# danielwillemsen/alphazero-openspiel

Measured on NVIDIA B200. Metric: mcts_simulations_per_sec, higher is better.
Workload: dtype f64

## Files before the change

alphazero_openspiel_b200/csrc/az_engine.cu:

```cuda

#include <cuda_runtime.h>
#include <cuda_bf16.h>
#include <stdint.h>
#include <stdio.h>
#include <stdarg.h>
#include <string.h>
#include <math.h>
#include <new>
#include <vector>

#include "../../include/az_b200.h"
#include "az_games.cuh"

namespace az {

constexpr int PH_BEGIN = 6;
constexpr int PH_COMPACT = 7;
constexpr int BLOCK = 128;
#ifndef K_STEP_MIN_BLOCKS
#define K_STEP_MIN_BLOCKS 7
#endif

struct __align__(16) TreeHdr {
  uint64_t root_b0, root_b1;
  uint64_t pend_b0, pend_b1;
  int32_t root_node;
  int32_t alloc;
  int32_t sims_done;
  int32_t pend_node;
  int32_t pend_depth;
  int32_t pend_ply;
  int32_t root_ply;
  int32_t game_seq;
  uint8_t phase, half, err, uct;
  int32_t fast_sims;
  int32_t pad2[2];
};
static_assert(sizeof(TreeHdr) == 80, "TreeHdr size");

__device__ __forceinline__ St root_state(const TreeHdr& h) {
  St s;
  s.b0 = h.root_b0;
  s.b1 = h.root_b1;
  s.ply = h.root_ply;
  return s;
}
__device__ __forceinline__ St pend_state(const TreeHdr& h) {
  St s;
  s.b0 = h.pend_b0;
  s.b1 = h.pend_b1;
  s.ply = h.pend_ply;
  return s;
}
__device__ __forceinline__ void set_root(TreeHdr& h, const St& s) {
  h.root_b0 = s.b0;
  h.root_b1 = s.b1;
  h.root_ply = s.ply;
}
__device__ __forceinline__ void set_pend(TreeHdr& h, const St& s, int node, int depth) {
  h.pend_b0 = s.b0;
  h.pend_b1 = s.b1;
  h.pend_ply = s.ply;
  h.pend_node = node;
  h.pend_depth = depth;
}

struct __align__(16) VlPend {
  uint64_t b0, b1;
  int32_t node, depth, ply, valid;
};

struct ResignCfg {
  double threshold;
  int32_t permille;
  int32_t pad;
};
struct ResignTree {
  double rmin[2];
  int32_t game_seq;
  int32_t calib;
};

struct PlayoutCapCfg {
  int32_t fast_playouts;
  int32_t full_permille;
};

struct Node;
struct Params {
  TreeHdr* hdr;
  Node* nodes;
  int32_t* path;
  uint8_t* rec;
  unsigned long long* rec_count;
  unsigned long long* ctr;
  int* games_started;
  int* compact_list;
  int* compact_count;
  long long* dbg;
  VlPend* vl_pend;
  int vl_k;
  uint8_t* cache;
  unsigned long long cache_mask;
  uint32_t* cache_epoch;
  ResignCfg* resign_cfg;
  ResignTree* resign_tree;
  PlayoutCapCfg* pcap_cfg;
  const double* logtab;
  long long rec_cap;
  int max_games;
  int rec_stride;
  int n_trees, cap;
  int n_playouts, num_prob, noise_mode, eval_mode, eval_shift, max_sims, start_mod;
  int cycle_budget;
  uint32_t flags;
  uint64_t seed;
  double c_puct, keep, noise_w, alpha, temperature;
  Geo geo;
};

__device__ __forceinline__ int search_target(const Params& p, const TreeHdr& h) {
  return h.fast_sims ? h.fast_sims : p.n_playouts;
}

struct StepIO {
  const void* priors;
  const void* values;
  const double* noise;
  void* obs;
  int obs_format;
};

template <int G>
__device__ __forceinline__ unsigned group_mask() {
  if constexpr (G >= 32) {
    return 0xffffffffu;
  } else {
    const unsigned lane = threadIdx.x & 31u;
    return ((1u << G) - 1u) << (lane & ~(unsigned)(G - 1));
  }
}
template <int G, class T>
__device__ __forceinline__ T gshfl(unsigned m, T v, int src) { return __shfl_sync(m, v, src, G); }
template <int G, class T>
__device__ __forceinline__ T gshfl_xor(unsigned m, T v, int off) { return __shfl_xor_sync(m, v, off, G); }
template <int G>
__device__ __forceinline__ int gsum(unsigned m, int v) {
#pragma unroll
  for (int o = G / 2; o > 0; o >>= 1) v += __shfl_xor_sync(m, v, o, G);
  return v;
}
template <int G>
__device__ __forceinline__ double gsumd(unsigned m, double v) {
#pragma unroll
  for (int o = G / 2; o > 0; o >>= 1) v += __shfl_xor_sync(m, v, o, G);
  return v;
}
template <int G>
__device__ __forceinline__ int gscan_incl(unsigned m, int v, int lane) {
#pragma unroll
  for (int o = 1; o < G; o <<= 1) {
    const int t = __shfl_up_sync(m, v, o, G);
    if (lane >= o) v += t;
  }
  return v;
}
template <int G>
__device__ __forceinline__ void gargmax(unsigned m, double& v, int& i) {
#pragma unroll
  for (int o = G / 2; o > 0; o >>= 1) {
    const double ov = __shfl_xor_sync(m, v, o, G);
    const int oi = __shfl_xor_sync(m, i, o, G);
    if (oi != 0x7fffffff && (i == 0x7fffffff || ov > v || (ov == v && oi < i))) { v = ov; i = oi; }
  }
}

__device__ __forceinline__ void ctr_add(unsigned long long* s_ctr, int which, unsigned long long v) {
  if (v) atomicAdd(&s_ctr[which], v);
}

struct StepCtr {
  unsigned long long sims = 0, depth = 0, children = 0, exp = 0, legal = 0, term = 0;
  __device__ __forceinline__ void flush(unsigned long long* s_ctr, int alloc) const {
    atomicMax(&s_ctr[AZ_CTR_PEAK_NODES], (unsigned long long)alloc);
    ctr_add(s_ctr, AZ_CTR_SIMS, sims);
    ctr_add(s_ctr, AZ_CTR_DEPTH, depth);
    ctr_add(s_ctr, AZ_CTR_CHILDREN, children);
    ctr_add(s_ctr, AZ_CTR_EXPANSIONS, exp);
    ctr_add(s_ctr, AZ_CTR_LEGAL, legal);
    ctr_add(s_ctr, AZ_CTR_TERMINAL, term);
  }
};

__device__ __forceinline__ void flush_block_counters(const Params& p, const unsigned long long* s_ctr) {
  __syncthreads();
  if (threadIdx.x < AZ_CTR_COUNT && s_ctr[threadIdx.x]) {
    if (threadIdx.x == AZ_CTR_PEAK_NODES) atomicMax(&p.ctr[threadIdx.x], s_ctr[threadIdx.x]);
    else atomicAdd(&p.ctr[threadIdx.x], s_ctr[threadIdx.x]);
  }
}

__device__ __forceinline__ void arena_overflow(TreeHdr& h, int lane, unsigned long long* s_ctr) {
  h.err = 1;
  if (lane == 0) ctr_add(s_ctr, AZ_CTR_OVERFLOW, 1);
}

struct EvalKey {
  uint64_t k;
};
__device__ __forceinline__ EvalKey eval_key(const Params& p, const St& s) {
  EvalKey e;
  e.k = mix64(s.b0 ^ mix64(s.b1 ^ mix64(p.seed + (uint64_t)(s.ply & 1))));
  return e;
}
__device__ __forceinline__ double eval_prior(const Params& p, const StepIO& io, int tree, const EvalKey& ek, int a) {
  if (p.eval_mode == AZ_EVAL_EXTERNAL) {
    const size_t idx = (size_t)tree * p.geo.n_actions + a;
    return (p.flags & AZ_F_PRIORS_F64) ? ((const double*)io.priors)[idx] : (double)((const float*)io.priors)[idx];
  }
  if (p.eval_mode == AZ_EVAL_UNIFORM) return 1.0 / (double)p.geo.n_actions;
  if (p.eval_mode == AZ_EVAL_ROLLOUT) return 1.0;
  const uint64_t ha = mix64(ek.k + (uint64_t)(a + 1) * 0xD1B54A32D192ED03ULL);
  return (double)(1 + (int)((ha >> 40) & 0x3FF)) * exp2((double)-(10 + p.eval_shift));
}
template <class GM>
__device__ double rollout_value(const Params& p, St s, const EvalKey& ek) {
  const int mover = s.ply & 1;
  for (uint64_t j = 0;; ++j) {
    const int out = GM::outcome(s, p.geo);
    if (out >= 0) return out == 2 ? 0.0 : (out == mover ? 1.0 : -1.0);
    const typename GM::Legal lg = GM::legal(s, p.geo);
    const int n = GM::count(lg);
    const uint64_t r = mix64(ek.k + (j + 1) * 0x9E3779B97F4A7C15ULL);
    s = GM::apply(s, p.geo, GM::action_of(lg, s, p.geo, (int)(r % (uint64_t)n)));
  }
}
template <class GM>
__device__ __forceinline__ double eval_value(const Params& p, const StepIO& io, int tree, const EvalKey& ek, const St& s) {
  if (p.eval_mode == AZ_EVAL_EXTERNAL)
    return (p.flags & AZ_F_PRIORS_F64) ? ((const double*)io.values)[tree] : (double)((const float*)io.values)[tree];
  if (p.eval_mode == AZ_EVAL_UNIFORM) return 0.0;
  if (p.eval_mode == AZ_EVAL_ROLLOUT) return rollout_value<GM>(p, s, ek);
  return (double)((int)((ek.k >> 20) & 31) - 16) / 16.0;
}

struct CacheHead {
  uint64_t b0, b1;
  uint32_t tag;
  float value;
};
static_assert(sizeof(CacheHead) == 24, "CacheHead size");
template <class GM>
__host__ __device__ constexpr int cache_stride() {
  int s = 1;
  while (s < (int)sizeof(CacheHead) + 4 * GM::MAXC + 4) s *= 2;
  return s;
}
template <class GM>
__device__ __forceinline__ uint8_t* cache_slot(const Params& p, const St& s) {
  return p.cache + (size_t)(eval_key(p, s).k & p.cache_mask) * cache_stride<GM>();
}
template <class GM>
__device__ __forceinline__ const CacheHead* cache_find(const Params& p, const St& s) {
  const CacheHead* e = reinterpret_cast<const CacheHead*>(cache_slot<GM>(p, s));
  const uint32_t tag = (p.cache_epoch[0] << 1) | (uint32_t)(s.ply & 1);
  return (e->b0 == s.b0 && e->b1 == s.b1 && e->tag == tag) ? e : nullptr;
}
__device__ __forceinline__ const float* cache_priors(const CacheHead* e) { return reinterpret_cast<const float*>(e + 1); }

__device__ double gamma_draw(double alpha, uint64_t seed, uint64_t tree, uint64_t gseq, uint64_t ply, int child) {
  const double d = alpha + 1.0 - 1.0 / 3.0, c = 1.0 / sqrt(9.0 * d);
  for (int att = 0; att < 64; ++att) {
    const uint64_t base = (uint64_t)child * 256 + (uint64_t)att * 4;
    const uint64_t r0 = counter(seed, tree, gseq, ply, base + 0, 5);
    const uint64_t r1 = counter(seed, tree, gseq, ply, base + 1, 5);
    const uint64_t r2 = counter(seed, tree, gseq, ply, base + 2, 5);
    const double u0 = ((double)(r0 >> 11) + 1.0) * (1.0 / 9007199254740992.0);
    const double u1 = ((double)(r1 >> 11) + 0.5) * (1.0 / 9007199254740992.0);
    const double u2 = ((double)(r2 >> 11) + 1.0) * (1.0 / 9007199254740992.0);
    const double x = sqrt(-2.0 * log(u0)) * cospi(2.0 * u1);
    double v = 1.0 + c * x;
    if (v <= 0.0) continue;
    v = v * v * v;
    const uint64_t r3 = counter(seed, tree, gseq, ply, base + 3, 5);
    const double u3 = ((double)(r3 >> 11) + 1.0) * (1.0 / 9007199254740992.0);
    if (log(u3) < 0.5 * x * x + d - d * v + d * log(v)) return d * v * pow(u2, 1.0 / alpha);
  }
  return alpha;
}

template <class GM, int G>
__device__ __forceinline__ void write_obs(const Params& p, const StepIO& io, int tree, int lane, const St& s) {
  if (io.obs_format == AZ_OBS_NONE || io.obs == nullptr) return;
  const int n = p.geo.cells;
  const uint64_t pl0 = GM::plane(s, p.geo, 0), pl1 = GM::plane(s, p.geo, 1), pl2 = GM::plane(s, p.geo, 2);
  const int cur = s.ply & 1;
  if (io.obs_format == AZ_OBS_BF16_NHWC) {
    uint2* out = reinterpret_cast<uint2*>(io.obs) + (size_t)tree * n;
    const uint32_t one = 0x3F80u;
    for (int c = lane; c < n; c += G) {
      uint2 v;
      v.x = (((pl0 >> c) & 1ULL) ? one : 0u) | ((((pl1 >> c) & 1ULL) ? one : 0u) << 16);
      v.y = (((pl2 >> c) & 1ULL) ? one : 0u) | ((cur ? one : 0u) << 16);
      out[c] = v;
    }
  } else {
    float* out = reinterpret_cast<float*>(io.obs) + (size_t)tree * 4 * n;
    for (int i = lane; i < 4 * n; i += G) {
      const int ch = i / n, c = i - ch * n;
      const uint64_t pm = ch == 0 ? pl0 : (ch == 1 ? pl1 : pl2);
      out[i] = ch == 3 ? (float)cur : (float)((pm >> c) & 1ULL);
    }
  }
}

struct __align__(8) Node {
  uint2 nl;
  double q;
  double p;
};
static_assert(sizeof(Node) == 24, "Node size");
struct Arena {
  Node* nd;
  __device__ __forceinline__ uint2& nl(int i) const { return nd[i].nl; }
  __device__ __forceinline__ double& q(int i) const { return nd[i].q; }
  __device__ __forceinline__ double& p(int i) const { return nd[i].p; }
};
__device__ __forceinline__ Arena arena_of(const Params& p, int tree, int half) {
  Arena a;
  a.nd = p.nodes + ((size_t)tree * 2 + half) * (size_t)p.cap;
  return a;
}

template <int G>
__device__ __forceinline__ void backup_path(const Arena& a, const int32_t* path, int depth, double v_leaf, int lane) {
  for (int j = lane; j <= depth; j += G) {
    const int node = path[j];
    const double v = ((depth - j) & 1) ? -v_leaf : v_leaf;
    const uint2 nl = a.nl(node);
    const double q = a.q(node);
    a.q(node) = __ddiv_rn(__dadd_rn(__dmul_rn((double)nl.x, q), v), (double)(nl.x + 1u));
    a.nl(node).x = nl.x + 1u;
  }
}

template <class GM, int G>
__device__ __forceinline__ bool expand_node(const Params& p, const StepIO& io, const Arena& a, TreeHdr& h, int tree,
                                            int node, const St& s, int lane, unsigned gm, bool root_mix,
                                            const double* eta_lane , int* L_out,
// ... 373 lines not shown
      const double ret0 = out == 2 ? 0.0 : (out == 0 ? 1.0 : -1.0);
      emit_record<GM, G>(p, tree, h, s2, 1, -1, 0, 0, ret0, rmin0, rmin1, end, nullptr, nullptr, lane, gm, s_ctr);
    }
    end_game<GM, G>(p, h, tree, lane, gm, s_ctr, s2);
    return;
  }
  set_root(h, s2);
  if ((p.flags & AZ_F_KEEP_TREE) && nc > 0) {
    if (!(p.flags & AZ_F_EAGER_COMPACT) && (long long)h.alloc + (long long)(p.n_playouts + 1) * GM::MAXC <= (long long)p.cap) {
      h.root_node = fc + k;
      h.phase = PH_BEGIN;
      return;
    }
    h.pend_node = fc + k;
    h.phase = PH_COMPACT;
    if (lane == 0) p.compact_list[atomicAdd(p.compact_count, 1)] = tree;
    return;
  }
  fresh_tree<G>(p, h, tree, lane, gm);
  h.phase = PH_BEGIN;
}

template <class GM, int G>
__device__ __forceinline__ void expand_root(const Params& p, const StepIO& io, TreeHdr& h, int tree, int row, int lane,
                                            unsigned gm, unsigned long long* s_ctr, const float* cached) {
  const Arena a = arena_of(p, tree, h.half);
  const St s = root_state(h);
  const typename GM::Legal lg = GM::legal(s, p.geo);
  const int L = GM::count(lg);
  double eta[GM::SLOTS];
#pragma unroll
  for (int sl = 0; sl < GM::SLOTS; ++sl) eta[sl] = 0.0;
  if (p.noise_mode == AZ_NOISE_HOST) {
#pragma unroll
    for (int sl = 0; sl < GM::SLOTS; ++sl) {
      const int i = lane + sl * G;
      if (i < L) eta[sl] = io.noise[(size_t)tree * GM::MAXC + i];
    }
  } else if (p.noise_mode == AZ_NOISE_COUNTER) {
    double sum = 0.0;
    for (int i = 0; i < L; ++i) {
      const double u = (double)((counter(p.seed, tree, h.game_seq, s.ply, i, 1) >> 11) + 1ULL) *
                       (1.0 / 9007199254740992.0);
      sum = __dadd_rn(sum, u);
#pragma unroll
      for (int sl = 0; sl < GM::SLOTS; ++sl)
        if (i == lane + sl * G) eta[sl] = u;
    }
#pragma unroll
    for (int sl = 0; sl < GM::SLOTS; ++sl) eta[sl] = __ddiv_rn(eta[sl], sum);
  } else if (p.noise_mode == AZ_NOISE_DIRICHLET) {
    double sum = 0.0;
#pragma unroll
    for (int sl = 0; sl < GM::SLOTS; ++sl) {
      const int i = lane + sl * G;
      if (i < L) eta[sl] = gamma_draw(p.alpha, p.seed, tree, h.game_seq, s.ply, i);
      sum += eta[sl];
    }
    sum = gsumd<G>(gm, sum);
#pragma unroll
    for (int sl = 0; sl < GM::SLOTS; ++sl) eta[sl] = sum > 0.0 ? eta[sl] / sum : 1.0 / (double)L;
  }
  int L2 = 0;
  if (!expand_node<GM, G>(p, io, a, h, row, h.root_node, s, lane, gm, true, eta, &L2, cached)) arena_overflow(h, lane, s_ctr);
  h.phase = AZ_PH_RUN;
  if (lane == 0) ctr_add(s_ctr, AZ_CTR_ROOT_EVALS, 1);
}

template <class GM, int G, bool CACHE>
__device__ __forceinline__ bool begin_search(const Params& p, const StepIO& io, TreeHdr& h, int tree, int row, int lane,
                                             unsigned gm, unsigned long long* s_ctr) {
  h.sims_done = 0;
  h.phase = AZ_PH_RUN;
  h.fast_sims = 0;
  if (p.flags & AZ_F_PLAYOUT_CAP) {
    const PlayoutCapCfg c = *p.pcap_cfg;
    if ((int)(counter(p.seed, tree, h.game_seq, h.root_ply, 0, 7) % 1000ULL) >= c.full_permille) {
      h.fast_sims = c.fast_playouts;
      return false;
    }
  }
  if (p.noise_mode == AZ_NOISE_NONE) return false;
  const St s = root_state(h);
  const CacheHead* hit = CACHE && p.cache ? cache_find<GM>(p, s) : nullptr;
  if (hit) {
    expand_root<GM, G>(p, io, h, tree, row, lane, gm, s_ctr, cache_priors(hit));
    return false;
  }
  h.phase = AZ_PH_ROOT_EVAL;
  set_pend(h, s, h.root_node, 0);
  write_obs<GM, G>(p, io, row, lane, s);
  return true;
}

template <class GM, int G, void (*BACKUP)(const Arena&, const int32_t*, int, double, int)>
__device__ __forceinline__ void apply_leaf(const Params& p, const StepIO& io, const Arena& a, TreeHdr& h, int row, int node,
                                           const St& s, const int32_t* path, int depth, const CacheHead* cached, int lane,
                                           unsigned gm, unsigned long long* s_ctr, StepCtr& c) {
  int L = 0;
  if (!expand_node<GM, G>(p, io, a, h, row, node, s, lane, gm, false, nullptr, &L, cached ? cache_priors(cached) : nullptr))
    arena_overflow(h, lane, s_ctr);
  const double v = cached ? (double)cached->value : eval_value<GM>(p, io, row, eval_key(p, s), s);
  BACKUP(a, path, depth, -v, lane);
  __syncwarp(gm);
  h.sims_done += 1;
  c.sims += 1;
  c.depth += depth;
  c.exp += 1;
  c.legal += L;
  if (cached && lane == 0) ctr_add(s_ctr, AZ_CTR_CACHE_HITS, 1);
}

template <int G>
__device__ __forceinline__ void terminal_leaf(const Arena& a, TreeHdr& h, const int32_t* path, int depth, int out, int ply,
                                              int lane, unsigned gm, StepCtr& c) {
  backup_path<G>(a, path, depth, mover_return(out, ply), lane);
  __syncwarp(gm);
  h.sims_done += 1;
  c.sims += 1;
  c.depth += depth;
  c.term += 1;
}

template <class GM, bool UCT>
__global__ void __launch_bounds__(BLOCK, K_STEP_MIN_BLOCKS) k_step(const Params p, const StepIO io) {
  constexpr int G = GM::G;
  __shared__ int32_t s_path[BLOCK / G][GM::MAXD];
  __shared__ unsigned long long s_ctr[AZ_CTR_COUNT];
  if (threadIdx.x < AZ_CTR_COUNT) s_ctr[threadIdx.x] = 0ULL;
  __syncthreads();
  const int tree = (int)((blockIdx.x * (unsigned)BLOCK + threadIdx.x) / G);
  const int lane = threadIdx.x % G;
  if (p.cache && blockIdx.x == 0 && threadIdx.x == 0) p.cache_epoch[1] = p.cache_epoch[0];
  if (tree < p.n_trees) {
    const unsigned gm = group_mask<G>();
    int32_t* spath = s_path[threadIdx.x / G];
    int32_t* gpath = p.path + (size_t)tree * GM::MAXD;
    const long long t_start = p.dbg ? clock64() : 0;
    const long long t_begin = p.cycle_budget > 0 ? clock64() : 0;
    TreeHdr h = p.hdr[tree];
    const int phase_in = h.phase;
    long long t_consume = 0;
    StepCtr c;

    if (h.phase == AZ_PH_LEAF_EVAL) {
      apply_leaf<GM, G, backup_path<G>>(p, io, arena_of(p, tree, h.half), h, tree, h.pend_node, pend_state(h), gpath,
                                        h.pend_depth, nullptr, lane, gm, s_ctr, c);
      h.phase = AZ_PH_RUN;
    } else if (h.phase == AZ_PH_ROOT_EVAL) {
      expand_root<GM, G>(p, io, h, tree, tree, lane, gm, s_ctr, nullptr);
    }

    if (p.dbg) t_consume = clock64() - t_start;
    int sims_this_step = 0;
    bool advanced = false;
    for (;;) {
      if (h.phase == PH_BEGIN && begin_search<GM, G, true>(p, io, h, tree, tree, lane, gm, s_ctr)) break;
      if (h.phase != AZ_PH_RUN) {
        if (lane == 0) ctr_add(s_ctr, AZ_CTR_IDLE_SLOTS, 1);
        break;
      }
      if (h.sims_done >= search_target(p, h)) {
        if (advanced) {
          if (lane == 0) ctr_add(s_ctr, AZ_CTR_IDLE_SLOTS, 1);
          break;
        }
        finish_move<GM, G>(p, h, tree, lane, gm, s_ctr);
        advanced = true;
        continue;
      }
      if (p.max_sims > 0 && sims_this_step >= p.max_sims) {
        if (lane == 0) ctr_add(s_ctr, AZ_CTR_IDLE_SLOTS, 1);
        break;
      }
      if (p.cycle_budget > 0 && sims_this_step > 0) {
        const int over = gshfl<G>(gm, (int)(clock64() - t_begin > (long long)p.cycle_budget), 0);
        if (over) {
          if (lane == 0) ctr_add(s_ctr, AZ_CTR_IDLE_SLOTS, 1);
          break;
        }
      }
      const Arena a = arena_of(p, tree, h.half);
      St s = root_state(h);
      int node, depth;
      bool dovf = false;
      sim_select<GM, G, UCT>(p, a, h.root_node, s, node, depth, spath, lane, gm, c.children, dovf, h.uct != 0);
      if (dovf) {
        h.err = 1;
        h.phase = AZ_PH_ERROR;
        if (lane == 0) ctr_add(s_ctr, AZ_CTR_OVERFLOW, 1);
        break;
      }
      const int out = depth > 0 ? GM::outcome(s, p.geo) : -1;
      ++sims_this_step;
      if (out >= 0) {
        terminal_leaf<G>(a, h, spath, depth, out, s.ply, lane, gm, c);
        if (p.flags & AZ_F_MANUAL) {
          for (int j = lane; j <= depth; j += G) gpath[j] = spath[j];
          h.pend_depth = depth;
        }
        continue;
      }
      const CacheHead* hit = p.cache ? cache_find<GM>(p, s) : nullptr;
      if (hit) {
        apply_leaf<GM, G, backup_path<G>>(p, io, a, h, tree, node, s, spath, depth, hit, lane, gm, s_ctr, c);
        continue;
      }
      set_pend(h, s, node, depth);
      h.phase = AZ_PH_LEAF_EVAL;
      for (int j = lane; j <= depth; j += G) gpath[j] = spath[j];
      write_obs<GM, G>(p, io, tree, lane, s);
      break;
    }

    if (lane == 0) {
      p.hdr[tree] = h;
      if (p.dbg) {
        p.dbg[4 * tree + 0] = clock64() - t_start;
        p.dbg[4 * tree + 1] = phase_in;
        p.dbg[4 * tree + 2] = sims_this_step;
        p.dbg[4 * tree + 3] = t_consume * 2 + (advanced ? 1 : 0);
      }
      c.flush(s_ctr, h.alloc);
    }
  }
  flush_block_counters(p, s_ctr);
}

template <class GM>
__global__ void __launch_bounds__(BLOCK) k_cache_insert(const Params p, const StepIO io) {
  constexpr int G = GM::G;
  const int tree = (int)((blockIdx.x * (unsigned)BLOCK + threadIdx.x) / G);
  const int lane = threadIdx.x % G;
  if (tree >= p.n_trees) return;
  const TreeHdr& h = p.hdr[tree];
  if (h.phase != AZ_PH_LEAF_EVAL && h.phase != AZ_PH_ROOT_EVAL) return;
  const unsigned gm = group_mask<G>();
  const St s = pend_state(h);
  uint8_t* slot = cache_slot<GM>(p, s);
  unsigned* lock = reinterpret_cast<unsigned*>(slot + cache_stride<GM>() - 4);
  int got = 0;
  if (lane == 0) got = atomicCAS(lock, 0u, 1u) == 0u;
  if (!gshfl<G>(gm, got, 0)) return;
  const typename GM::Legal lg = GM::legal(s, p.geo);
  const int L = GM::count(lg);
  float* pri = reinterpret_cast<float*>(slot + sizeof(CacheHead));
  const float* row = (const float*)io.priors + (size_t)tree * p.geo.n_actions;
#pragma unroll
  for (int sl = 0; sl < GM::SLOTS; ++sl) {
    const int i = lane + sl * G;
    if (i < L) pri[i] = row[GM::action_of(lg, s, p.geo, i)];
  }
  if (lane == 0) {
    CacheHead e;
    e.b0 = s.b0;
    e.b1 = s.b1;
    e.tag = (p.cache_epoch[1] << 1) | (uint32_t)(s.ply & 1);
    e.value = ((const float*)io.values)[tree];
    *reinterpret_cast<CacheHead*>(slot) = e;
  }
  __threadfence();
  __syncwarp(gm);
  if (lane == 0) atomicExch(lock, 0u);
}

__global__ void k_cache_new_epoch(uint32_t* epoch) { epoch[0] += 1u; }

constexpr unsigned VL_MARK = 0xFFFFFF00u;

template <int G>
__device__ __forceinline__ void vl_apply(const Arena& a, const int32_t* path, int depth, int lane) {
  for (int j = lane; j <= depth; j += G) {
    const int node = path[j];
    const uint2 nl = a.nl(node);
    a.q(node) = ((double)nl.x * a.q(node) - 1.0) / (double)(nl.x + 1u);
    a.nl(node).x = nl.x + 1u;
  }
}
template <int G>
__device__ __forceinline__ void vl_backup(const Arena& a, const int32_t* path, int depth, double v_leaf, int lane) {
  for (int j = lane; j <= depth; j += G) {
    const int node = path[j];
    const double v = ((depth - j) & 1) ? -v_leaf : v_leaf;
    const uint2 nl = a.nl(node);
    a.q(node) = ((double)nl.x * a.q(node) + 1.0 + v) / (double)nl.x;
  }
}

template <class GM>
__global__ void __launch_bounds__(BLOCK, 4) k_step_vl(const Params p, const StepIO io) {
  constexpr int G = GM::G;
  __shared__ int32_t s_path[BLOCK / G][GM::MAXD];
  __shared__ unsigned long long s_ctr[AZ_CTR_COUNT];
  if (threadIdx.x < AZ_CTR_COUNT) s_ctr[threadIdx.x] = 0ULL;
  __syncthreads();
  const int tree = (int)((blockIdx.x * (unsigned)BLOCK + threadIdx.x) / G);
  const int lane = threadIdx.x % G;
  if (tree < p.n_trees) {
    const unsigned gm = group_mask<G>();
    const int K = p.vl_k;
    int32_t* spath = s_path[threadIdx.x / G];
    int32_t* gpaths = p.path + (size_t)tree * K * GM::MAXD;
    VlPend* pend = p.vl_pend + (size_t)tree * K;
    const int row0 = tree * K;
    TreeHdr h = p.hdr[tree];
    StepCtr c;

    if (h.phase == AZ_PH_LEAF_EVAL) {
      const Arena a = arena_of(p, tree, h.half);
      for (int slot = 0; slot < K; ++slot) {
        const VlPend pe = pend[slot];
        if (!pe.valid) continue;
        St s;
        s.b0 = pe.b0;
        s.b1 = pe.b1;
        s.ply = pe.ply;
        if (lane == 0) a.nl(pe.node).y = 0u;
        __syncwarp(gm);
        apply_leaf<GM, G, vl_backup<G>>(p, io, a, h, row0 + slot, pe.node, s, gpaths + (size_t)slot * GM::MAXD, pe.depth,
                                        nullptr, lane, gm, s_ctr, c);
        if (lane == 0) pend[slot].valid = 0;
      }
      h.phase = AZ_PH_RUN;
    } else if (h.phase == AZ_PH_ROOT_EVAL) {
      expand_root<GM, G>(p, io, h, tree, row0, lane, gm, s_ctr, nullptr);
    }

    int n_pending = 0, sims_this_step = 0;
    bool advanced = false;
    for (;;) {
      if (h.phase == PH_BEGIN && begin_search<GM, G, false>(p, io, h, tree, row0, lane, gm, s_ctr)) {
        n_pending = 1;
        break;
      }
      if (h.phase != AZ_PH_RUN) break;
      if (h.sims_done + n_pending >= search_target(p, h)) {
        if (n_pending > 0 || advanced) break;
        finish_move<GM, G>(p, h, tree, lane, gm, s_ctr);
        advanced = true;
        continue;
      }
      if (n_pending >= K) break;
      if (p.max_sims > 0 && sims_this_step >= p.max_sims + K) break;
      const Arena a = arena_of(p, tree, h.half);
      St s = root_state(h);
      int node, depth;
      bool dovf = false;
      sim_select<GM, G, false>(p, a, h.root_node, s, node, depth, spath, lane, gm, c.children, dovf, false);
      if (dovf) {
// ... 426 lines not shown
  for (int r = 0; r < rows; ++r) {
    c0 |= 1ULL << (r * cols);
    cl |= 1ULL << (r * cols + cols - 1);
  }
  g.notcol0 = g.all & ~c0;
  g.notcolL = g.all & ~cl;
  g.row0 = cols >= 64 ? ~0ULL : ((1ULL << cols) - 1ULL);
  g.rowL = g.row0 << ((rows - 1) * cols);
  return g;
}

static int check_game(int game_id, int rows, int cols) {
  if (game_id == AZ_GAME_CONNECT_FOUR) return 0;
  if (game_id != AZ_GAME_BREAKTHROUGH) return fail(-1, "unknown game_id %d", game_id);
  if (rows < 4 || cols < 2 || rows * cols > 64 || cols > 16)
    return fail(-1, "breakthrough %dx%d unsupported (need rows>=4, cols>=2, rows*cols<=64)", rows, cols);
  return 0;
}

template <class F>
static int dispatch_game(int game_id, F&& f) {
  if (game_id == AZ_GAME_CONNECT_FOUR) return f(C4());
  return f(BT());
}

static inline int compact_grid(int n_trees) {
  int grid = n_trees / 128 + 4;
  return grid > 296 ? 296 : grid;
}
static inline int groups_grid(int n_trees, int G, int block) { return (int)(((long long)n_trees * G + block - 1) / block); }

extern "C" {

const char* az_last_error(void) { return g_err; }
int az_version(void) { return 1; }

int az_create(const az_config* cfg_in, az_engine** out) {
  if (!cfg_in || !out) return fail(-1, "null argument");
  az_config cfg = *cfg_in;
  if (check_game(cfg.game_id, cfg.rows, cfg.cols)) return -1;
  if (cfg.game_id == AZ_GAME_CONNECT_FOUR) {
    cfg.rows = 6;
    cfg.cols = 7;
  }
  if (cfg.n_trees <= 0) return fail(-1, "n_trees must be positive");
  if (cfg.n_playouts <= 0) return fail(-1, "n_playouts must be positive");
  if (cfg.temperature <= 0.0) cfg.temperature = 1.0;
  if (cfg.dirichlet_alpha <= 0.0) cfg.dirichlet_alpha = 0.3;
  if (cfg.noise_weight == 0.0) cfg.noise_weight = 0.25;
  if (cfg.num_probabilistic_actions <= 0) cfg.num_probabilistic_actions = 1000;
  if (cfg.noise_mode < 0 || cfg.noise_mode > 3) return fail(-1, "bad noise_mode");
  if (cfg.eval_mode < 0 || cfg.eval_mode > 3) return fail(-1, "bad eval_mode");
  const int maxc = cfg.game_id == AZ_GAME_CONNECT_FOUR ? C4::MAXC : BT::MAXC;
  const int maxd = cfg.game_id == AZ_GAME_CONNECT_FOUR ? C4::MAXD : BT::MAXD;
  const int group = cfg.game_id == AZ_GAME_CONNECT_FOUR ? C4::G : BT::G;
  if (cfg.node_capacity <= 0) {
    const int branch = cfg.game_id == AZ_GAME_CONNECT_FOUR ? 7 : 3 * cfg.cols + 8;
    long long c = (long long)(cfg.n_playouts + 2) * branch * 8 + 64;
    if (c > (1 << 24) - 1) c = (1 << 24) - 1;
    cfg.node_capacity = (int)c;
  }
  if (cfg.node_capacity >= (1 << 24)) return fail(-1, "node_capacity must be < 2^24");
  if (cfg.leaves_per_tree <= 0 || !(cfg.flags & AZ_F_VIRTUAL_LOSS)) cfg.leaves_per_tree = 1;
  if (cfg.leaves_per_tree > 64) return fail(-1, "leaves_per_tree must be <= 64");
  if ((cfg.flags & AZ_F_VIRTUAL_LOSS) && (cfg.flags & (AZ_F_MANUAL | AZ_F_UCT)))
    return fail(-1, "AZ_F_VIRTUAL_LOSS is a batched self-play mode (no AZ_F_MANUAL / AZ_F_UCT)");
  if ((cfg.flags & AZ_F_RESIGN) && (cfg.flags & AZ_F_MANUAL))
    return fail(-1, "AZ_F_RESIGN is a batched self-play mode: with AZ_F_MANUAL the host decides the moves");
  if ((cfg.flags & AZ_F_PLAYOUT_CAP) && (cfg.flags & AZ_F_MANUAL))
    return fail(-1, "AZ_F_PLAYOUT_CAP is a batched self-play mode: with AZ_F_MANUAL the host starts the searches");
  if (cfg.record_capacity <= 0) cfg.record_capacity = cfg.n_trees * 64 < (1 << 20) ? (1 << 20) : cfg.n_trees * 64;
  if (!(cfg.flags & AZ_F_RECORDS)) cfg.record_capacity = 1;
  if (cfg.flags & AZ_F_EVAL_CACHE) {
    if (cfg.eval_mode != AZ_EVAL_EXTERNAL || (cfg.flags & (AZ_F_PRIORS_F64 | AZ_F_MANUAL | AZ_F_VIRTUAL_LOSS)) ||
        cfg.noise_mode == AZ_NOISE_HOST)
      return fail(-1, "AZ_F_EVAL_CACHE needs AZ_EVAL_EXTERNAL float outputs, no AZ_F_MANUAL / AZ_F_VIRTUAL_LOSS / "
                      "AZ_NOISE_HOST");
    int lg = (int)AZ_EVAL_CACHE_LOG2(cfg.flags);
    if (lg == 0) {
      lg = AZ_EVAL_CACHE_EXTRA_LOG2;
      while ((1LL << lg) < (long long)cfg.n_trees * cfg.n_playouts << AZ_EVAL_CACHE_EXTRA_LOG2) ++lg;
      lg = lg < 16 ? 16 : (lg > 27 ? 27 : lg);
    }
    if (lg > 30) return fail(-1, "evaluator cache size 2^%d: at most 2^30 entries", lg);
    cfg.flags = (cfg.flags & ~(31u << AZ_EVAL_CACHE_LOG2_SHIFT)) | ((uint32_t)lg << AZ_EVAL_CACHE_LOG2_SHIFT);
  } else {
    cfg.flags &= ~(31u << AZ_EVAL_CACHE_LOG2_SHIFT);
  }

  CK(cudaSetDevice(cfg.device));
  cudaDeviceProp prop;
  CK(cudaGetDeviceProperties(&prop, cfg.device));
  if (prop.major < 10) return fail(-3, "az_b200 needs an sm_100a GPU (found sm_%d%d)", prop.major, prop.minor);

  az_engine* e = new (std::nothrow) az_engine();
  if (!e) return fail(-4, "out of host memory");
  memset(e, 0, sizeof(*e));
  e->cfg = cfg;
  e->max_children = maxc;
  e->maxd = maxd;
  e->group = group;
  Params& p = e->p;
  p.n_trees = cfg.n_trees;
  p.cap = cfg.node_capacity;
  p.n_playouts = cfg.n_playouts;
  p.num_prob = cfg.num_probabilistic_actions;
  p.noise_mode = cfg.noise_mode;
  p.eval_mode = cfg.eval_mode;
  p.eval_shift = cfg.eval_shift;
  p.max_sims = cfg.max_sims_per_step;
  p.cycle_budget = cfg.step_cycle_budget > 0 ? cfg.step_cycle_budget : 0;
  p.start_mod = cfg.start_plies_mod;
  p.flags = cfg.flags;
  p.seed = cfg.seed;
  p.c_puct = cfg.c_puct;
  p.keep = 1.0 - cfg.dirichlet_ratio;
  p.noise_w = cfg.noise_weight;
  p.alpha = cfg.dirichlet_alpha;
  p.temperature = cfg.temperature;
  p.geo = make_geo(cfg.game_id, cfg.rows, cfg.cols);
  p.rec_stride = (int)((sizeof(az_record) + 6 * (size_t)maxc + 7) / 8 * 8);
  p.max_games = cfg.max_games;
  p.rec_cap = cfg.record_capacity;
  p.vl_k = cfg.leaves_per_tree;

  const size_t nodes = (size_t)cfg.n_trees * 2 * (size_t)cfg.node_capacity;
  size_t bytes = 0;
  auto alloc = [&](void** ptr, size_t n) -> cudaError_t {
    bytes += n;
    return cudaMalloc(ptr, n);
  };
  cudaError_t err = cudaSuccess;
  if ((err = alloc((void**)&p.hdr, sizeof(TreeHdr) * (size_t)cfg.n_trees)) != cudaSuccess ||
      (err = alloc((void**)&p.nodes, sizeof(Node) * nodes)) != cudaSuccess ||
      (err = alloc((void**)&p.path, sizeof(int32_t) * (size_t)cfg.n_trees * maxd * (size_t)cfg.leaves_per_tree)) != cudaSuccess ||
      (err = alloc((void**)&p.vl_pend, sizeof(VlPend) * (size_t)cfg.n_trees * (size_t)cfg.leaves_per_tree)) != cudaSuccess ||
      (err = alloc((void**)&p.rec, (size_t)p.rec_stride * (size_t)p.rec_cap)) != cudaSuccess ||
      (err = alloc((void**)&p.rec_count, sizeof(unsigned long long))) != cudaSuccess ||
      (err = alloc((void**)&p.ctr, sizeof(unsigned long long) * AZ_CTR_COUNT)) != cudaSuccess ||
      (err = alloc((void**)&p.games_started, sizeof(int))) != cudaSuccess ||
      (err = alloc((void**)&p.compact_list, sizeof(int) * (size_t)cfg.n_trees)) != cudaSuccess ||
      (err = alloc((void**)&p.compact_count, sizeof(int) * 2)) != cudaSuccess ||
      (err = alloc((void**)&e->d_cmd, sizeof(int32_t) * ((size_t)cfg.n_trees * 3))) != cudaSuccess ||
      (err = alloc((void**)&e->d_bad, sizeof(int32_t))) != cudaSuccess) {
    fail(-2, "cudaMalloc failed (%zu bytes requested so far): %s", bytes, cudaGetErrorString(err));
    az_destroy(e);
    return -2;
  }
  if (cfg.flags & AZ_F_EVAL_CACHE) {
    const size_t n = (size_t)1 << AZ_EVAL_CACHE_LOG2(cfg.flags);
    const size_t cbytes = n * (cfg.game_id == AZ_GAME_CONNECT_FOUR ? cache_stride<C4>() : cache_stride<BT>());
    if ((err = alloc((void**)&p.cache, cbytes)) != cudaSuccess ||
        (err = alloc((void**)&p.cache_epoch, 2 * sizeof(uint32_t))) != cudaSuccess) {
      fail(-2, "cudaMalloc failed (evaluator cache, %zu bytes): %s", cbytes, cudaGetErrorString(err));
      az_destroy(e);
      return -2;
    }
    p.cache_mask = n - 1;
    const uint32_t epoch0[2] = {1u, 1u};
    CK(cudaMemset(p.cache, 0, cbytes));
    CK(cudaMemcpy(p.cache_epoch, epoch0, sizeof(epoch0), cudaMemcpyHostToDevice));
  }
  if (cfg.flags & AZ_F_RESIGN) {
    if ((err = alloc((void**)&p.resign_cfg, sizeof(ResignCfg))) != cudaSuccess ||
        (err = alloc((void**)&p.resign_tree, sizeof(ResignTree) * (size_t)cfg.n_trees)) != cudaSuccess) {
      fail(-2, "cudaMalloc failed (resignation state): %s", cudaGetErrorString(err));
      az_destroy(e);
      return -2;
    }
    const ResignCfg rc0 = {-1.0, 0, 0};
    CK(cudaMemcpy(p.resign_cfg, &rc0, sizeof(rc0), cudaMemcpyHostToDevice));
  }
  if (cfg.flags & AZ_F_PLAYOUT_CAP) {
    if ((err = alloc((void**)&p.pcap_cfg, sizeof(PlayoutCapCfg))) != cudaSuccess) {
      fail(-2, "cudaMalloc failed (playout cap): %s", cudaGetErrorString(err));
      az_destroy(e);
      return -2;
    }
    const PlayoutCapCfg pc0 = {cfg.n_playouts, 1000};
    CK(cudaMemcpy(p.pcap_cfg, &pc0, sizeof(pc0), cudaMemcpyHostToDevice));
  }
  if (cfg.flags & AZ_F_UCT) {
    double* tab = nullptr;
    if ((err = alloc((void**)&tab, sizeof(double) * LOGTAB_N)) != cudaSuccess) {
      fail(-2, "cudaMalloc failed (log table): %s", cudaGetErrorString(err));
      az_destroy(e);
      return -2;
    }
    p.logtab = tab;
    std::vector<double> host(LOGTAB_N);
    for (int n = 0; n < LOGTAB_N; ++n) host[n] = log((double)n);
    CK(cudaMemcpy(tab, host.data(), sizeof(double) * LOGTAB_N, cudaMemcpyHostToDevice));
  }
  e->bytes = (int64_t)bytes;
  CK(cudaMemset(p.rec_count, 0, sizeof(unsigned long long)));
  CK(cudaMemset(p.ctr, 0, sizeof(unsigned long long) * AZ_CTR_COUNT));
  CK(cudaMemset(e->d_bad, 0, sizeof(int32_t)));
  CK(cudaMemset(p.compact_count, 0, sizeof(int) * 2));
  CK(cudaMemset(p.vl_pend, 0, sizeof(VlPend) * (size_t)cfg.n_trees * (size_t)cfg.leaves_per_tree));
  *out = e;
  int rc = az_reset(e, nullptr);
  if (rc) return rc;
  CK(cudaDeviceSynchronize());
  return 0;
}

int az_destroy(az_engine* e) {
  if (!e) return 0;
  Params& p = e->p;
  cudaFree(p.hdr);
  cudaFree(p.nodes);
  cudaFree(p.path);
  cudaFree(p.vl_pend);
  cudaFree(p.rec);
  cudaFree(p.rec_count);
  cudaFree(p.ctr);
  cudaFree(p.games_started);
  cudaFree(p.compact_list);
  cudaFree(p.compact_count);
  if (p.dbg) cudaFree(p.dbg);
  if (p.logtab) cudaFree(const_cast<double*>(p.logtab));
  if (p.cache) cudaFree(p.cache);
  if (p.cache_epoch) cudaFree(p.cache_epoch);
  if (p.resign_cfg) cudaFree(p.resign_cfg);
  if (p.resign_tree) cudaFree(p.resign_tree);
  if (p.pcap_cfg) cudaFree(p.pcap_cfg);
  cudaFree(e->d_cmd);
  cudaFree(e->d_bad);
  delete e;
  return 0;
}

int az_config_get(const az_engine* e, az_config* out) {
  if (!e || !out) return fail(-1, "null argument");
  *out = e->cfg;
  return 0;
}
int az_max_children(const az_engine* e) { return e ? e->max_children : -1; }
int az_num_actions(const az_engine* e) { return e ? e->p.geo.n_actions : -1; }
int az_record_stride(const az_engine* e) { return e ? e->p.rec_stride : -1; }
int64_t az_device_bytes(const az_engine* e) { return e ? e->bytes : -1; }

int az_reset(az_engine* e, void* stream) {
  if (!e) return fail(-1, "null engine");
  cudaStream_t st = (cudaStream_t)stream;
  const Params p = e->p;
  CK(cudaMemcpyAsync(p.games_started, &e->cfg.n_trees, sizeof(int), cudaMemcpyHostToDevice, st));
  CK(cudaMemsetAsync(p.compact_count, 0, sizeof(int) * 2, st));
  if (p.resign_tree) CK(cudaMemsetAsync(p.resign_tree, 0xff, sizeof(ResignTree) * (size_t)p.n_trees, st));
  dispatch_game(e->cfg.game_id, [&](auto gm) {
    using GM = decltype(gm);
    k_reset<GM><<<groups_grid(p.n_trees, GM::G, BLOCK), BLOCK, 0, st>>>(p);
    return 0;
  });
  CK(cudaGetLastError());
  return 0;
}

static int check_bad(az_engine* e, cudaStream_t st, const char* what) {
  int32_t bad = 0;
  CK(cudaMemcpyAsync(&bad, e->d_bad, sizeof(bad), cudaMemcpyDeviceToHost, st));
  CK(cudaStreamSynchronize(st));
  if (bad) {
    cudaMemsetAsync(e->d_bad, 0, sizeof(int32_t), st);
    return fail(-5, "%s: %d tree(s) got an illegal action", what, bad);
  }
  return 0;
}

int az_set_positions(az_engine* e, const int32_t* hist_host, const int32_t* len_host, int32_t max_len, void* stream) {
  if (!e || !len_host) return fail(-1, "null argument");
  cudaStream_t st = (cudaStream_t)stream;
  const Params p = e->p;
  const size_t hn = (size_t)p.n_trees * (size_t)(max_len > 0 ? max_len : 1);
  int32_t* d_tmp = nullptr;
  CK(cudaMalloc((void**)&d_tmp, sizeof(int32_t) * (hn + (size_t)p.n_trees)));
  int32_t *d_len = d_tmp, *d_hist = d_tmp + p.n_trees;
  struct Free {
    int32_t* ptr;
    ~Free() { cudaFree(ptr); }
  } guard{d_tmp};
  if (max_len > 0 && hist_host) CK(cudaMemcpyAsync(d_hist, hist_host, sizeof(int32_t) * hn, cudaMemcpyHostToDevice, st));
  CK(cudaMemcpyAsync(d_len, len_host, sizeof(int32_t) * (size_t)p.n_trees, cudaMemcpyHostToDevice, st));
  dispatch_game(e->cfg.game_id, [&](auto gm) {
    using GM = decltype(gm);
    k_set_positions<GM><<<(p.n_trees + 127) / 128, 128, 0, st>>>(p, d_hist, d_len, max_len > 0 ? max_len : 1, e->d_bad);
    return 0;
  });
  CK(cudaGetLastError());
  return check_bad(e, st, "az_set_positions");
}

int az_command(az_engine* e, const int32_t* update_root_host, const int32_t* reset_tree_host, const int32_t* begin_host,
               void* stream) {
  if (!e) return fail(-1, "null engine");
  cudaStream_t st = (cudaStream_t)stream;
  const Params p = e->p;
  const size_t n = (size_t)p.n_trees;
  int32_t* d_upd = update_root_host ? e->d_cmd : nullptr;
  int32_t* d_rst = reset_tree_host ? e->d_cmd + n : nullptr;
  int32_t* d_beg = begin_host ? e->d_cmd + 2 * n : nullptr;
  if (d_upd) CK(cudaMemcpyAsync(d_upd, update_root_host, sizeof(int32_t) * n, cudaMemcpyHostToDevice, st));
  if (d_rst) CK(cudaMemcpyAsync(d_rst, reset_tree_host, sizeof(int32_t) * n, cudaMemcpyHostToDevice, st));
  if (d_beg) CK(cudaMemcpyAsync(d_beg, begin_host, sizeof(int32_t) * n, cudaMemcpyHostToDevice, st));
  dispatch_game(e->cfg.game_id, [&](auto gm) {
    using GM = decltype(gm);
    k_command<GM><<<groups_grid(p.n_trees, GM::G, BLOCK), BLOCK, 0, st>>>(p, d_upd, d_rst, d_beg, e->d_bad);
    return 0;
  });
  if (d_upd) k_compact<<<compact_grid(p.n_trees), 256, 0, st>>>(p);
  CK(cudaGetLastError());
  return check_bad(e, st, "az_command(update_root)");
}

int az_step(az_engine* e, const void* priors_dev, const void* values_dev, const double* noise_dev, void* obs_dev,
            int32_t obs_format, void* stream) {
  if (!e) return fail(-1, "null engine");
  if (obs_format < 0 || obs_format > 2) return fail(-1, "bad obs_format");
  cudaStream_t st = (cudaStream_t)stream;
  const Params p = e->p;
  StepIO io;
  io.priors = priors_dev;
  io.values = values_dev;
  io.noise = noise_dev;
  io.obs = obs_dev;
  io.obs_format = obs_format;
  if (p.noise_mode == AZ_NOISE_HOST && !noise_dev) return fail(-1, "AZ_NOISE_HOST needs noise_dev");
  if ((p.flags & AZ_F_KEEP_TREE) && !(p.flags & AZ_F_MANUAL) && !(p.flags & AZ_F_ASYNC_COMPACT)) {
    k_compact<<<compact_grid(p.n_trees), 256, 0, st>>>(p);
    CK(cudaGetLastError());
  }
  dispatch_game(e->cfg.game_id, [&](auto gm) {
    using GM = decltype(gm);
    if (p.cache && priors_dev) k_cache_insert<GM><<<groups_grid(p.n_trees, GM::G, BLOCK), BLOCK, 0, st>>>(p, io);
    if (p.flags & AZ_F_VIRTUAL_LOSS) k_step_vl<GM><<<groups_grid(p.n_trees, GM::G, BLOCK), BLOCK, 0, st>>>(p, io);
    else if (p.flags & AZ_F_UCT) k_step<GM, true><<<groups_grid(p.n_trees, GM::G, BLOCK), BLOCK, 0, st>>>(p, io);
    else k_step<GM, false><<<groups_grid(p.n_trees, GM::G, BLOCK), BLOCK, 0, st>>>(p, io);
    return 0;
  });
  CK(cudaGetLastError());
  return 0;
}

int az_eval_cache_invalidate(az_engine* e, void* stream) {
  if (!e) return fail(-1, "null engine");
  if (!e->p.cache) return 0;
  k_cache_new_epoch<<<1, 1, 0, (cudaStream_t)stream>>>(e->p.cache_epoch);
  CK(cudaGetLastError());
  return 0;
}

int az_set_resign(az_engine* e, double threshold, int32_t disabled_permille, void* stream) {
  if (!e) return fail(-1, "null engine");
  if (!e->p.resign_cfg) return fail(-1, "az_set_resign: the engine was created without AZ_F_RESIGN");
  if (!isfinite(threshold)) return fail(-1, "az_set_resign: the threshold must be finite");
  if (disabled_permille < 0 || disabled_permille > 1000)
    return fail(-1, "az_set_resign: disabled_permille %d is outside [0, 1000]", disabled_permille);
  const ResignCfg rc = {threshold, disabled_permille, 0};
  CK(cudaMemcpyAsync(e->p.resign_cfg, &rc, sizeof(rc), cudaMemcpyHostToDevice, (cudaStream_t)stream));
  return 0;
}

int az_set_playout_cap(az_engine* e, int32_t fast_playouts, int32_t full_permille, void* stream) {
  if (!e) return fail(-1, "null engine");
  if (!e->p.pcap_cfg) return fail(-1, "az_set_playout_cap: the engine was created without AZ_F_PLAYOUT_CAP");
  if (fast_playouts < 1 || fast_playouts > e->p.n_playouts)
    return fail(-1, "az_set_playout_cap: fast_playouts %d is outside [1, n_playouts = %d]", fast_playouts, e->p.n_playouts);
  if (full_permille < 0 || full_permille > 1000)
    return fail(-1, "az_set_playout_cap: full_permille %d is outside [0, 1000]", full_permille);
  const PlayoutCapCfg pc = {fast_playouts, full_permille};
  CK(cudaMemcpyAsync(e->p.pcap_cfg, &pc, sizeof(pc), cudaMemcpyHostToDevice, (cudaStream_t)stream));
  return 0;
}

int az_compact(az_engine* e, void* stream) {
  if (!e) return fail(-1, "null engine");
  const Params p = e->p;
  k_compact<<<compact_grid(p.n_trees), 256, 0, (cudaStream_t)stream>>>(p);
  CK(cudaGetLastError());
  return 0;
}

int az_debug_timing(az_engine* e, long long* out_host) {
  if (!e || !out_host) return fail(-1, "null argument");
  const size_t bytes = sizeof(long long) * 4 * (size_t)e->p.n_trees;
  if (!e->p.dbg) {
    CK(cudaMalloc((void**)&e->p.dbg, bytes));
    CK(cudaMemset(e->p.dbg, 0, bytes));
  }
  CK(cudaMemcpy(out_host, e->p.dbg, bytes, cudaMemcpyDeviceToHost));
  return 0;
}

int az_status(az_engine* e, int32_t* phase_dev, int32_t* sims_dev, int32_t* ply_dev, int32_t* req_legal_dev, void* stream) {
  if (!e) return fail(-1, "null engine");
  const Params p = e->p;
  dispatch_game(e->cfg.game_id, [&](auto gm) {
    using GM = decltype(gm);
    k_status<GM><<<(p.n_trees + 127) / 128, 128, 0, (cudaStream_t)stream>>>(p, phase_dev, sims_dev, ply_dev, req_legal_dev);
    return 0;
  });
  CK(cudaGetLastError());
  return 0;
}

int az_request_info(az_engine* e, uint64_t* bb_dev, int32_t* ply_dev, int32_t* path_actions_dev, int32_t* depth_dev,
                    int32_t max_depth, void* stream) {
  if (!e) return fail(-1, "null engine");
  const Params p = e->p;
  dispatch_game(e->cfg.game_id, [&](auto gm) {
    using GM = decltype(gm);
    k_request_info<GM><<<(p.n_trees + 127) / 128, 128, 0, (cudaStream_t)stream>>>(p, bb_dev, ply_dev, path_actions_dev,
                                                                                 depth_dev, max_depth);
    return 0;
  });
  CK(cudaGetLastError());
  return 0;
}

int az_root_stats(az_engine* e, int32_t* root_n_dev, double* root_q_dev, int32_t* n_children_dev, int32_t* child_action_dev,
                  int32_t* child_n_dev, double* child_q_dev, double* child_p_dev, double* v_a0c_dev,
                  double* v_offpolicy_dev, void* stream) {
  if (!e) return fail(-1, "null engine");
  const Params p = e->p;
  dispatch_game(e->cfg.game_id, [&](auto gm) {
    using GM = decltype(gm);
    k_root_stats<GM><<<groups_grid(p.n_trees, GM::G, BLOCK), BLOCK, 0, (cudaStream_t)stream>>>(
        p, root_n_dev, root_q_dev, n_children_dev, child_action_dev, child_n_dev, child_q_dev, child_p_dev, v_a0c_dev,
        v_offpolicy_dev);
    return 0;
// ... 88 lines not shown
```

Baseline: 44.11 million.

## Make evaluator cache 4-way set-associative with stamp-based replacement

Replaces the direct-mapped evaluator cache with 4-way buckets, probed in parallel by group lanes using a ballot. Insertion picks a victim by rank (same key, stale epoch, then age via a per-round stamp) and claims it with a CAS on the stamp, replacing the per-slot spin lock. The goal is fewer conflict misses, and so fewer external evaluations per simulation, plus cheaper locking. The cost is extra probe loads and ballots on every lookup, and a racier write protocol with no fence.

```diff
diff --git a/alphazero_openspiel_b200/csrc/az_engine.cu b/alphazero_openspiel_b200/csrc/az_engine.cu
--- a/alphazero_openspiel_b200/csrc/az_engine.cu
+++ b/alphazero_openspiel_b200/csrc/az_engine.cu
@@ -102,7 +102,7 @@
   int vl_k;
   uint8_t* cache;
   unsigned long long cache_mask;
-  uint32_t* cache_epoch;
+  uint32_t* cache_ctl;
   ResignCfg* resign_cfg;
   ResignTree* resign_tree;
   PlayoutCapCfg* pcap_cfg;
@@ -145,6 +145,12 @@
 template <int G, class T>
 __device__ __forceinline__ T gshfl_xor(unsigned m, T v, int off) { return __shfl_xor_sync(m, v, off, G); }
 template <int G>
+__device__ __forceinline__ unsigned group_ballot(unsigned m, bool pred) {
+  const unsigned b = __ballot_sync(m, pred);
+  if constexpr (G >= 32) return b;
+  else return (b >> ((threadIdx.x & 31u) & ~(unsigned)(G - 1))) & ((1u << G) - 1u);
+}
+template <int G>
 __device__ __forceinline__ int gsum(unsigned m, int v) {
 #pragma unroll
   for (int o = G / 2; o > 0; o >>= 1) v += __shfl_xor_sync(m, v, o, G);
@@ -244,27 +250,41 @@
   return (double)((int)((ek.k >> 20) & 31) - 16) / 16.0;
 }
 
+constexpr int CACHE_WAYS = 4;
 struct CacheHead {
   uint64_t b0, b1;
   uint32_t tag;
   float value;
+  uint32_t stamp;
+  uint32_t pad;
 };
-static_assert(sizeof(CacheHead) == 24, "CacheHead size");
+static_assert(sizeof(CacheHead) == 32, "CacheHead size");
 template <class GM>
 __host__ __device__ constexpr int cache_stride() {
   int s = 1;
-  while (s < (int)sizeof(CacheHead) + 4 * GM::MAXC + 4) s *= 2;
+  while (s < (int)sizeof(CacheHead) + 4 * GM::MAXC) s *= 2;
   return s;
 }
 template <class GM>
-__device__ __forceinline__ uint8_t* cache_slot(const Params& p, const St& s) {
-  return p.cache + (size_t)(eval_key(p, s).k & p.cache_mask) * cache_stride<GM>();
-}
-template <class GM>
-__device__ __forceinline__ const CacheHead* cache_find(const Params& p, const St& s) {
-  const CacheHead* e = reinterpret_cast<const CacheHead*>(cache_slot<GM>(p, s));
-  const uint32_t tag = (p.cache_epoch[0] << 1) | (uint32_t)(s.ply & 1);
-  return (e->b0 == s.b0 && e->b1 == s.b1 && e->tag == tag) ? e : nullptr;
+__device__ __forceinline__ uint8_t* cache_bucket(const Params& p, const St& s) {
+  return p.cache + (size_t)(eval_key(p, s).k & p.cache_mask) * (CACHE_WAYS * cache_stride<GM>());
+}
+template <class GM, int G>
+__device__ __forceinline__ const CacheHead* cache_find(const Params& p, const St& s, int lane, unsigned gm) {
+  uint8_t* b = cache_bucket<GM>(p, s);
+  bool match = false;
+  if (lane < CACHE_WAYS) {
+    const CacheHead* e = reinterpret_cast<const CacheHead*>(b + lane * cache_stride<GM>());
+    const ulonglong2 k = *reinterpret_cast<const ulonglong2*>(e);
+    const uint32_t tag = (p.cache_ctl[0] << 1) | (uint32_t)(s.ply & 1);
+    match = k.x == s.b0 && k.y == s.b1 && e->tag == tag;
+  }
+  const unsigned hits = group_ballot<G>(gm, match);
+  if (!hits) return nullptr;
+  const int w = __ffs(hits) - 1;
+  CacheHead* e = reinterpret_cast<CacheHead*>(b + w * cache_stride<GM>());
+  if (lane == w) e->stamp = p.cache_ctl[3];
+  return e;
 }
 __device__ __forceinline__ const float* cache_priors(const CacheHead* e) { return reinterpret_cast<const float*>(e + 1); }
 
@@ -804,7 +824,7 @@
   }
   if (p.noise_mode == AZ_NOISE_NONE) return false;
   const St s = root_state(h);
-  const CacheHead* hit = CACHE && p.cache ? cache_find<GM>(p, s) : nullptr;
+  const CacheHead* hit = CACHE && p.cache ? cache_find<GM, G>(p, s, lane, gm) : nullptr;
   if (hit) {
     expand_root<GM, G>(p, io, h, tree, row, lane, gm, s_ctr, cache_priors(hit));
     return false;
@@ -853,7 +873,10 @@
   __syncthreads();
   const int tree = (int)((blockIdx.x * (unsigned)BLOCK + threadIdx.x) / G);
   const int lane = threadIdx.x % G;
-  if (p.cache && blockIdx.x == 0 && threadIdx.x == 0) p.cache_epoch[1] = p.cache_epoch[0];
+  if (p.cache && blockIdx.x == 0 && threadIdx.x == 0) {
+    p.cache_ctl[1] = p.cache_ctl[0];
+    p.cache_ctl[2] = p.cache_ctl[3] + 1u;
+  }
   if (tree < p.n_trees) {
     const unsigned gm = group_mask<G>();
     int32_t* spath = s_path[threadIdx.x / G];
@@ -923,7 +946,7 @@
         }
         continue;
       }
-      const CacheHead* hit = p.cache ? cache_find<GM>(p, s) : nullptr;
+      const CacheHead* hit = p.cache ? cache_find<GM, G>(p, s, lane, gm) : nullptr;
       if (hit) {
         apply_leaf<GM, G, backup_path<G>>(p, io, a, h, tree, node, s, spath, depth, hit, lane, gm, s_ctr, c);
         continue;
@@ -954,16 +977,45 @@
   constexpr int G = GM::G;
   const int tree = (int)((blockIdx.x * (unsigned)BLOCK + threadIdx.x) / G);
   const int lane = threadIdx.x % G;
+  const uint32_t round = p.cache_ctl[2];
+  if (blockIdx.x == 0 && threadIdx.x == 0) p.cache_ctl[3] = round;
   if (tree >= p.n_trees) return;
   const TreeHdr& h = p.hdr[tree];
   if (h.phase != AZ_PH_LEAF_EVAL && h.phase != AZ_PH_ROOT_EVAL) return;
   const unsigned gm = group_mask<G>();
   const St s = pend_state(h);
-  uint8_t* slot = cache_slot<GM>(p, s);
-  unsigned* lock = reinterpret_cast<unsigned*>(slot + cache_stride<GM>() - 4);
-  int got = 0;
-  if (lane == 0) got = atomicCAS(lock, 0u, 1u) == 0u;
-  if (!gshfl<G>(gm, got, 0)) return;
+  uint8_t* const bucket = cache_bucket<GM>(p, s);
+  unsigned long long score = ~0ULL;
+  uint32_t stamp = 0;
+  bool dup = false;
+  if (lane < CACHE_WAYS) {
+    const CacheHead c = *reinterpret_cast<const CacheHead*>(bucket + lane * cache_stride<GM>());
+    const bool same = c.b0 == s.b0 && c.b1 == s.b1 && (c.tag & 1u) == (uint32_t)(s.ply & 1);
+    const unsigned long long rank = same ? 0 : (c.tag >> 1) != p.cache_ctl[1] ? 1 : 2;
+    stamp = c.stamp;
+    dup = same && stamp == round;
+    if (stamp != round) score = rank << 32 | (unsigned long long)(uint32_t)~(round - stamp);
+  }
+  if (group_ballot<G>(gm, dup)) return;
+  int way = -1;
+  for (int t = 0; t < CACHE_WAYS && way < 0; ++t) {
+    unsigned long long best = score;
+#pragma unroll
+    for (int o = 1; o < CACHE_WAYS; o <<= 1) best = min(best, gshfl_xor<G>(gm, best, o));
+    best = gshfl<G>(gm, best, 0);
+    if (best == ~0ULL) return;
+    const int w = __ffs(group_ballot<G>(gm, lane < CACHE_WAYS && score == best)) - 1;
+    int got = 0;
+    if (lane == w) {
+      got = atomicCAS(reinterpret_cast<uint32_t*>(bucket + w * cache_stride<GM>() + offsetof(CacheHead, stamp)), stamp,
+                      round) == stamp;
+      score = ~0ULL;
+    }
+    if (gshfl<G>(gm, got, w)) way = w;
+    else if ((best >> 32) == 0) return;
+  }
+  if (way < 0) return;
+  uint8_t* const slot = bucket + way * cache_stride<GM>();
   const typename GM::Legal lg = GM::legal(s, p.geo);
   const int L = GM::count(lg);
   float* pri = reinterpret_cast<float*>(slot + sizeof(CacheHead));
@@ -974,19 +1026,15 @@
     if (i < L) pri[i] = row[GM::action_of(lg, s, p.geo, i)];
   }
   if (lane == 0) {
-    CacheHead e;
-    e.b0 = s.b0;
-    e.b1 = s.b1;
-    e.tag = (p.cache_epoch[1] << 1) | (uint32_t)(s.ply & 1);
-    e.value = ((const float*)io.values)[tree];
-    *reinterpret_cast<CacheHead*>(slot) = e;
-  }
-  __threadfence();
-  __syncwarp(gm);
-  if (lane == 0) atomicExch(lock, 0u);
-}
-
-__global__ void k_cache_new_epoch(uint32_t* epoch) { epoch[0] += 1u; }
+    CacheHead* e = reinterpret_cast<CacheHead*>(slot);
+    e->b0 = s.b0;
+    e->b1 = s.b1;
+    e->tag = (p.cache_ctl[1] << 1) | (uint32_t)(s.ply & 1);
+    e->value = ((const float*)io.values)[tree];
+  }
+}
+
+__global__ void k_cache_new_epoch(uint32_t* ctl) { ctl[0] += 1u; }
 
 constexpr unsigned VL_MARK = 0xFFFFFF00u;
 
@@ -1579,7 +1627,7 @@
       while ((1LL << lg) < (long long)cfg.n_trees * cfg.n_playouts << AZ_EVAL_CACHE_EXTRA_LOG2) ++lg;
       lg = lg < 16 ? 16 : (lg > 27 ? 27 : lg);
     }
-    if (lg > 30) return fail(-1, "evaluator cache size 2^%d: at most 2^30 entries", lg);
+    if (lg < 2 || lg > 30) return fail(-1, "evaluator cache size 2^%d: 2^2 (one bucket) to 2^30 entries", lg);
     cfg.flags = (cfg.flags & ~(31u << AZ_EVAL_CACHE_LOG2_SHIFT)) | ((uint32_t)lg << AZ_EVAL_CACHE_LOG2_SHIFT);
   } else {
     cfg.flags &= ~(31u << AZ_EVAL_CACHE_LOG2_SHIFT);
@@ -1648,15 +1696,15 @@
     const size_t n = (size_t)1 << AZ_EVAL_CACHE_LOG2(cfg.flags);
     const size_t cbytes = n * (cfg.game_id == AZ_GAME_CONNECT_FOUR ? cache_stride<C4>() : cache_stride<BT>());
     if ((err = alloc((void**)&p.cache, cbytes)) != cudaSuccess ||
-        (err = alloc((void**)&p.cache_epoch, 2 * sizeof(uint32_t))) != cudaSuccess) {
+        (err = alloc((void**)&p.cache_ctl, 4 * sizeof(uint32_t))) != cudaSuccess) {
       fail(-2, "cudaMalloc failed (evaluator cache, %zu bytes): %s", cbytes, cudaGetErrorString(err));
       az_destroy(e);
       return -2;
     }
-    p.cache_mask = n - 1;
-    const uint32_t epoch0[2] = {1u, 1u};
+    p.cache_mask = n / CACHE_WAYS - 1;
+    const uint32_t ctl0[4] = {1u, 1u, 1u, 0u};
     CK(cudaMemset(p.cache, 0, cbytes));
-    CK(cudaMemcpy(p.cache_epoch, epoch0, sizeof(epoch0), cudaMemcpyHostToDevice));
+    CK(cudaMemcpy(p.cache_ctl, ctl0, sizeof(ctl0), cudaMemcpyHostToDevice));
   }
   if (cfg.flags & AZ_F_RESIGN) {
     if ((err = alloc((void**)&p.resign_cfg, sizeof(ResignCfg))) != cudaSuccess ||
@@ -1718,7 +1766,7 @@
   if (p.dbg) cudaFree(p.dbg);
   if (p.logtab) cudaFree(const_cast<double*>(p.logtab));
   if (p.cache) cudaFree(p.cache);
-  if (p.cache_epoch) cudaFree(p.cache_epoch);
+  if (p.cache_ctl) cudaFree(p.cache_ctl);
   if (p.resign_cfg) cudaFree(p.resign_cfg);
   if (p.resign_tree) cudaFree(p.resign_tree);
   if (p.pcap_cfg) cudaFree(p.pcap_cfg);
@@ -1842,7 +1890,7 @@
 int az_eval_cache_invalidate(az_engine* e, void* stream) {
   if (!e) return fail(-1, "null engine");
   if (!e->p.cache) return 0;
-  k_cache_new_epoch<<<1, 1, 0, (cudaStream_t)stream>>>(e->p.cache_epoch);
+  k_cache_new_epoch<<<1, 1, 0, (cudaStream_t)stream>>>(e->p.cache_ctl);
   CK(cudaGetLastError());
   return 0;
 }
```

New measurement: 44.97 million (median of 6 runs). 1.02x the previous value.
